# tkkiran/Robust-Conditional-GAN

Hardware: AMD Instinct MI355X
Metric: images/sec G+D train step (CIFAR-10 RCGAN bs=64) (higher is better)
Workload: dtype bf16

## Files before the change

### robust-conditional-gan_amd/cifar.py

```python
import ctypes as C
import os

import warnings

import numpy as np
import torch

from . import _lib as L
from . import ops as O
from .ops_cifar import NO_OPS, Conv2D, Linear, cond_batchnorm, embed_y, spectral_normed_weight
from .runtime import DT, Context, ParamGroup, check_f32_matmul_precision
from .variables import Graph, scoped, variable_scope

Z_DIM = 128
DIM_G = 128
DIM_D = 128
VOCAB_SIZE = 10
EMBEDDING_DIM = 300
IMG_SIZE = 32
IMG_DIM = 3
OUTPUT_DIM = 3072
N_CRITIC = 5
GEN_BS_MULTIPLE = 2
ALGORITHMS = ("rcgan", "rcgan-u", "biased", "unbiased")
# ... 481 lines not shown
            for name, shp, dt in self.feed_layout["d" if steps is not None else key]:
                n = int(np.prod(shp))
                a = np.asarray(arrs[name]).reshape(-1)
                if dt == L.F32:
                    dst[off:off + n].view(np.float32)[:] = a
                else:
                    dst[off:off + n] = a
                off += n
        assert off == words, (off, words)
        with torch.cuda.stream(self.ctx.stream):
            self.feed[key].copy_(ring["slots"][i], non_blocking=True)
            ev = torch.cuda.Event()
            ev.record(self.ctx.stream)
        ring["events"][i] = ev

    def set_feed(self, key, blob):
        src = blob if isinstance(blob, torch.Tensor) else torch.from_numpy(np.ascontiguousarray(blob, dtype=np.int32))
        if src.is_cuda and src.dtype == torch.int32 and src.is_contiguous() and FEED_COPY_KERNEL:
            ctx = self.ctx
            assert src.numel() == self.feed[key].numel(), (src.numel(), self.feed[key].numel())
            ctx.check(ctx.lib.rcgan_copy_words(ctx.h, src.numel(), C.c_void_p(src.data_ptr()), C.c_void_p(self.feed[key].data_ptr())))
            return
        with torch.cuda.stream(self.ctx.stream):
            self.feed[key].copy_(src.reshape(-1), non_blocking=True)

    def _rng(self, t, kind, lo, hi):
        ctx = self.ctx
        ctx.check(ctx.lib.rcgan_rng_fill(ctx.h, t.size, t.dtype, kind, lo, hi, self.seed * 1000003 + self.rank,
                                         C.c_void_p(self.rng_state.data_ptr()), C.c_void_p(t.ptr)))

    def _draw_aug(self, u):
        if self.device_rng:
            ctx = self.ctx
            ctx.check(ctx.lib.rcgan_rng_fill(ctx.h, u.size, u.dtype, 0, 0.0, 1.0, self.seed * 1000003 + self.rank + 700001,
                                             C.c_void_p(self.aug_rng_state.data_ptr()), C.c_void_p(u.ptr)))
        return u

    def _sn_entries(self, conv_update, proj_update):
        ents = []
        for name in self.PD.names:
            if name.endswith("/Filters"):
                ents.append((name, name[:-len("Filters")] + "filters/spectral_norm/u", conv_update))
            elif name.endswith("/W"):
                base = name[:-2]
                upd = conv_update if base.endswith("D.Output") else proj_update
                ents.append((name, base + "/spectral_norm/u", upd))
        return ents

    def _filter_names(self, grp):
        names = []
        pool = fused_pool_d(self.ctx, GEN_BS_MULTIPLE * self.B)
        for n in grp.names:
            if n.endswith("/Filters"):
                shp = grp.shapes[n]
                up = L.CONV_IN_UPSAMPLE2X if (n.startswith("Generator/G.Block.") and n.endswith(".Conv1/Filters")) else 0
                if pool and n in ("Discriminator/D.Block.1.Conv2/Filters", "Discriminator/D.Block.2.Conv2/Filters"):
                    up = L.CONV_OUT_MEANPOOL2
                names.append((n, shp[0], 1, IMG_SIZE if min(shp[2], shp[3]) <= 3 else 8, up))
            elif n == "Generator/G.Input/W" and O.LINEAR_MFMA:
                names.append((n, 1, 1, 1, 0))
        return names

    def _prepare_all(self, which, head_update=False, inputs=None):
        names = []
        for grp in which:
            if grp is not self.PG:
                names += self._filter_names(grp)
        g, embed = self.graph, None
        g.head_E = None
        if self.fused_head and self.PD in which and head_update is not False and self.K <= L.LABELS_NARROW and \
                os.environ.get("RCGAN_HEAD_EMBED_RIDE", "1") == "1":
            _, _, table, w_e, b_e = _head_weights(head_update)
            E = self.ctx.empty((table.shape[0], w_e.param.shape[-1]), L.F32)
            embed = (table, w_e, b_e, E)
        g.trunk_frag = None
        trunk, rf = None, []
        if self.PD in which and self.ctx.act_dtype != L.F32 and (FUSED_TRUNK or O.RF_CONV):
            sn = lambda n: g.sn["Discriminator/%s/Filters" % n][0]
            trunk = [sn("D.Block.%d.%s" % (b, c)) for b in (3, 4, 5, 6) for c in ("Conv1", "Conv2")] if FUSED_TRUNK else None
            if O.RF_CONV:
                d = L.ConvDesc(1, 16, 16, DIM_D, DIM_D, 3, 3, 1, self.ctx.act_dtype, L.CONV_IN_RELU)
                if self.ctx.lib.rcgan_conv_rf_ok(C.byref(d)):
                    rf.append((sn("D.Block.2.Conv1"), d))
        if (trunk or rf) and O.FRAG_IN_PREPARE:
            tf, reqs = O.fragment_requests(self.ctx, trunk, rf)
            rode, written = g.prepare_convs(names, self.ctx.act_dtype, embed=embed, inputs=inputs, frags=reqs)
            if len(written) == len(reqs):
                g.trunk_frag = tf
            else:
                g.trunk_frag = O.fragments_batch(self.ctx, trunk, rf)
        else:
            rode = g.prepare_convs(names, self.ctx.act_dtype, embed=embed, inputs=inputs)
            if trunk or rf:
                g.trunk_frag = O.fragments_batch(self.ctx, trunk, rf)
        if rode and embed is not None:
            g.head_E = embed[3]
        return rode

    def _refresh_generator_filters(self):
        if self._pg_prepared_version != self.PG.version:
            self.graph.refresh_persistent(self._filter_names(self.PG), self.ctx.act_dtype)
            self._pg_prepared_version = self.PG.version

    def confusion_matrix(self):
        ctx = self.ctx
        if self.PC is not None:
            return O.softmax_rows(ctx, self.graph.param("confusion_logits"))
        return self.inp["C_const"]

    def _rides_inputs(self):
        return self.device_rng and self.ride_inputs and self.PD.gradbuf.numel() % 4 == 0

    def _d_body(self, fakes_ready=False):
        ctx, g, B, inp = self.ctx, self.graph, self.B, self.inp
        self._refresh_generator_filters()
        ctx.new_step()
        g.begin_step({1})
        ctx.sn_adam = (dict(group=self.PD, beta1=0.0, beta2=0.9, grad_scale=1.0 / (self.world * self.loss_scale))
                       if (self.fused_tail and ctx.recording and self.PD.hyper is not None) else None)
        g.early_d = self._dp_early(self.PD) if (self.dp_overlap and ctx.recording) else None
        ride = fakes_ready and self._rides_inputs()
        x_all = self.x_all if fakes_ready else ctx.empty((2 * B, OUTPUT_DIM))
        real, fake_dst = x_all.rows(0, B), x_all.rows(B, 2 * B)
        si = None
        if ride:
            fptr, fcount = self.PD.zero_grad(defer=True)
            g.image_pool = ctx.empty((2 * B, 16, 16, 3), x_all.dtype)
            si = L.StepInputsDesc(B, real.dtype, inp["images"].ptr, x_all.ptr, g.image_pool.ptr,
                                  0.0, 1.0 / 128, self.seed * 1000003 + self.rank, self.rng_state.data_ptr(), fptr, fcount,
                                  self.fakes_all.ptr, self.slice_ctr.data_ptr(), N_CRITIC)
        else:
            g.image_pool = None
            self.PD.zero_grad()
            if self.device_rng:
                self._rng(inp["noise"], 0, 0.0, 1.0 / 128)
                if not fakes_ready:
                    self._rng(inp["z"], 1, 0.0, 1.0)
        g.prefetch_sn(self._sn_entries(True, True))
        rode = self._prepare_all((self.PD,) if fakes_ready else (self.PG, self.PD), head_update=None, inputs=si)
        assert rode or si is None, "the step-input rider needs the batched filter preparation"
        if si is None:
            ctx.check(ctx.lib.rcgan_preprocess_cifar(ctx.h, B, inp["images"].ptr, inp["noise"].ptr, real.dtype, real.ptr))
        if fakes_ready:
            fake = self.x_all.rows(B, 2 * B)
        else:
            fake = Generator(B, inp["labels_random"], inp["z"], out=fake_dst)
        d_in = x_all
        if self.aug:
            d_in, g.image_pool = O.diffaugment(ctx, x_all, self._draw_aug(inp["aug_u"]), self.aug, pool=True)
        w = 1.0
        if self.fused_head:
            feat = Discriminator(d_in, None, update_collection=None, _head=False)
            lab_r, lab_f = inp["labels_all"].rows(0, B), inp["labels_all"].rows(B, 2 * B)
            if self.alg == "rcgan-u":
                y_conf = O.gather_rows(ctx, self.confusion_matrix(), inp["labels_random"], B)
                parts = [(B, L.LOSS_HINGE_REAL, inp["labels"], None), (B, L.LOSS_HINGE_FAKE, None, y_conf)]
            elif self.alg == "unbiased":
                parts = [(B, L.LOSS_HINGE_REAL, None, inp["inv_weights"]), (B, L.LOSS_HINGE_FAKE, inp["labels_random"], None)]
            else:
                parts = [(B, L.LOSS_HINGE_REAL, lab_r, None), (B, L.LOSS_HINGE_FAKE, lab_f, None)]
            Discriminator_head(feat, parts, w, self.loss_d, update_collection=None, logits=self.head_logits)
        elif self.alg == "rcgan-u":
            feat_a, wgan_a = Discriminator(d_in, None, update_collection=None)
            feat, wgan = O.rows(ctx, feat_a, 0, B), O.rows(ctx, wgan_a, 0, B)
            feat_f, wgan_f = O.rows(ctx, feat_a, B, 2 * B), O.rows(ctx, wgan_a, B, 2 * B)
            emb = Discriminator_projection(inp["labels"], update_collection=None)
            disc_real = O.proj_logit(ctx, feat, wgan, emb)
            E = Discriminator_projection(inp["arange"], update_collection=None)
            disc_fake = O.proj_logit_all(ctx, feat_f, wgan_f, E)
            y_conf = O.gather_rows(ctx, self.confusion_matrix(), inp["labels_random"], B)
            O.loss_term(ctx, L.LOSS_HINGE_FAKE, disc_fake, w, self.loss_d, wts=y_conf)
            O.loss_term(ctx, L.LOSS_HINGE_REAL, disc_real, w, self.loss_d)
        else:
            feat, wgan = Discriminator(d_in, None, update_collection=None)
            if self.alg in ("biased", "rcgan"):
                emb = Discriminator_projection(inp["labels_all"], update_collection=None)
                disc_all = O.proj_logit(ctx, feat, wgan, emb)
# ... 462 lines not shown
```

### robust-conditional-gan_amd/csrc/conv_mfma.hip

```cpp
#include <vector>
#include "conv_mfma.h"
#include "small_gemm.h"
#include "step_inputs.h"
#include "mfma_util.h"
#include "conv_image.h"
#include "head_rider.h"

#define LDS_PITCH 72
#define WG_PITCH 144



__device__ __forceinline__ void decode_pix(long m, int H, int W, int lh, int lw, int& n, int& oh, int& ow) {
  if (lw >= 0 && lh >= 0) {
    const unsigned mm = (unsigned)m;
    ow = (int)(mm & (unsigned)(W - 1));
    oh = (int)((mm >> lw) & (unsigned)(H - 1));
    n = (int)(mm >> (lw + lh));
  } else {
    ow = (int)(m % W);
    long t = m / W;
    oh = (int)(t % H);
    n = (int)(t / H);
  }
// ... 1037 lines not shown
  long r = idx / Cout;
  int ci = (int)(r % Cin);
  int t = (int)(r / Cin);
  bf16_t v = f32_to_bf16(w[idx] * inv);
  wt[(long)co * T * Cin + (long)t * Cin + ci] = v;
  wd[(long)ci * T * Cout + (long)(T - 1 - t) * Cout + co] = v;
}

struct PhasePrepBatch { struct It { const float* w; const float* sigma; bf16_t* wph; int Cin, Cout, kind; } it[8]; };
__device__ __forceinline__ void phase_taps2(int kind, int ph, int a, int& k0, int& k1) {
  if (kind == 0) { k0 = ph == 0 ? (a == 0 ? 0 : 1) : (a == 0 ? 0 : 2); k1 = ph == 0 ? (a == 0 ? 0 : 2) : (a == 0 ? 1 : 2); }
  else {
    const int u = ph == 0 ? (a == 0 ? 3 : 1) : (a == 0 ? 2 : 0);
    k0 = u == 0 ? 0 : (u == 1 ? 0 : (u == 2 ? 1 : 2)); k1 = u == 0 ? 0 : (u == 1 ? 1 : 2);
  }
}
__device__ __forceinline__ void phase_taps4(int kind, int u, int& k0, int& k1) {
  if (kind == 0) { k0 = u == 0 ? 2 : (u == 1 ? 1 : 0); k1 = u == 0 ? 2 : (u == 1 ? 2 : (u == 2 ? 1 : 0)); }
  else { k0 = u == 0 ? 0 : (u == 1 ? 0 : (u == 2 ? 1 : 2)); k1 = u == 0 ? 0 : (u == 1 ? 1 : 2); }
}

__global__ __launch_bounds__(256) void conv_prepare_phase_kernel(PhasePrepBatch b) {
  const PhasePrepBatch::It it = b.it[blockIdx.y];
  const float inv = (it.sigma ? 1.f / *it.sigma : 1.f) * (it.kind == 1 ? 0.25f : 1.f);
  const long total = 16L * it.Cin * it.Cout;
  bf16_t* const phase_l = it.kind == 0 ? it.wph : it.wph + total;
  bf16_t* const gather_l = it.kind == 0 ? it.wph + total : it.wph;
  const bool fwd_is_phase = it.kind == 0;
  const int Op = fwd_is_phase ? it.Cout : it.Cin, Rp = fwd_is_phase ? it.Cin : it.Cout;
  const int Og = fwd_is_phase ? it.Cin : it.Cout, Rg = fwd_is_phase ? it.Cout : it.Cin;
  for (long e = (long)blockIdx.x * blockDim.x + threadIdx.x; e < total; e += (long)gridDim.x * blockDim.x) {
    {
      const long per = (long)Op * 4 * Rp;
      const int phase = (int)(e / per);
      long r = e - phase * per;
      const int o = (int)(r / (4 * Rp));
      r -= (long)o * 4 * Rp;
      const int ab = (int)(r / Rp), rr = (int)(r - (long)ab * Rp);
      int kh0, kh1, kw0, kw1;
      phase_taps2(it.kind, phase >> 1, ab >> 1, kh0, kh1);
      phase_taps2(it.kind, phase & 1, ab & 1, kw0, kw1);
      const int ci = fwd_is_phase ? rr : o, co = fwd_is_phase ? o : rr;
      float s = 0.f;
      for (int kh = kh0; kh <= kh1; ++kh)
        for (int kw = kw0; kw <= kw1; ++kw) s += it.w[(((long)kh * 3 + kw) * it.Cin + ci) * it.Cout + co];
      phase_l[e] = f32_to_bf16(s * inv);
    }
    {
      const int o = (int)(e / (16L * Rg));
      long r = e - (long)o * 16 * Rg;
      const int uv = (int)(r / Rg), rr = (int)(r - (long)uv * Rg);
      int kh0, kh1, kw0, kw1;
      phase_taps4(it.kind, uv >> 2, kh0, kh1);
      phase_taps4(it.kind, uv & 3, kw0, kw1);
      const int ci = fwd_is_phase ? o : rr, co = fwd_is_phase ? rr : o;
      float s = 0.f;
      for (int kh = kh0; kh <= kh1; ++kh)
        for (int kw = kw0; kw <= kw1; ++kw) s += it.w[(((long)kh * 3 + kw) * it.Cin + ci) * it.Cout + co];
      gather_l[e] = f32_to_bf16(s * inv);
    }
  }
}

int conv_prepare_phase_launch(rcgan_ctx* ctx, int n, const float* const* ws, const float* const* sigmas, bf16_t* const* outs, const int* cins, const int* couts,
                              const int* kinds) {
  for (int base = 0; base < n; base += 8) {
    PhasePrepBatch b;
    const int m = n - base < 8 ? n - base : 8;
    long maxel = 0;
    for (int i = 0; i < m; ++i) {
      b.it[i] = {ws[base + i], sigmas[base + i], outs[base + i], cins[base + i], couts[base + i], kinds[base + i]};
      const long el = 16L * cins[base + i] * couts[base + i];
      if (el > maxel) maxel = el;
    }
    int bx = (int)cdiv(maxel, 256 * 8);
    if (bx > 1024) bx = 1024;
    hipLaunchKernelGGL(conv_prepare_phase_kernel, dim3(bx, m), dim3(256), 0, ctx->stream, b);
    RC_LAUNCH_CHECK(ctx);
  }
  return RCGAN_OK;
}

struct PrepItem { const float* w; const float* sigma; void* out; void* extra; int T, Cin, Cout, mfma, img; };
struct FragRow { int item; int ctn, ss; bf16_t* fwd; bf16_t* bwd; };
struct PrepBatch { PrepItem it[48]; PhasePrepBatch::It ph[8]; FragRow fr[12]; int start[72]; int n, rows, frag_row0, nfrag, gemm_row, inputs_row; SmallGemmArgs gemm; StepInputsArgs inputs; };

static_assert(sizeof(PrepBatch) <= 4096, "kernel arguments are limited to 4 KiB");
constexpr int PREP_MAX_ROWS = (int)(sizeof(PrepBatch::it) / sizeof(PrepItem) + sizeof(PrepBatch::ph) / sizeof(PhasePrepBatch::It) +
                                    sizeof(PrepBatch::fr) / sizeof(FragRow)) + 2;
constexpr int PREP_ROW_STEP = 64;
static_assert(PREP_MAX_ROWS <= 2 * PREP_ROW_STEP, "the row search must reach every row a launch can hold");
static_assert(PREP_MAX_ROWS + 1 <= (int)(sizeof(PrepBatch::start) / sizeof(int)), "start[] holds rows + 1 entries");

__device__ __forceinline__ long frag_index(int row, int k, int ctn, int ss, int nsl) {
  const int blk = row / (16 * ctn), ct = (row - blk * 16 * ctn) >> 4, r = row & 15;
  const int ks = k >> 5, sl = ks / ss, s = ks - sl * ss, kc = (k >> 3) & 3, e = k & 7;
  return ((((long)(blk * nsl + sl) * ss + s) * ctn + ct) * 64 + kc * 16 + r) * 8 + e;
}

__device__ __forceinline__ void prepare_fragment_units(const PrepItem& it, const FragRow& fr, bf16_t (*tile)[66], int bid, int nb) {
  const float inv = it.sigma ? 1.f / *it.sigma : 1.f;
  const int nci = it.Cin / 64, nco = it.Cout / 64;
  const int ntiles = it.T * nci * nco;
  const int nsl_f = it.T * it.Cin / 32 / fr.ss, nsl_d = it.T * it.Cout / 32 / fr.ss;
  const int lane64 = threadIdx.x & 63, grp = threadIdx.x >> 6;
  for (int tl = bid; tl < ntiles; tl += nb) {
    const int cot = tl % nco, cit = (tl / nco) % nci, t = tl / (nco * nci);
    const int ci0 = cit * 64, co0 = cot * 64;
    __syncthreads();
    float v[16];
#pragma unroll
    for (int i = 0; i < 16; ++i) v[i] = it.w[((long)t * it.Cin + ci0 + i * 4 + grp) * it.Cout + co0 + lane64];
#pragma unroll
    for (int i = 0; i < 16; ++i) {
      const int ci = i * 4 + grp;
      const bf16_t h = f32_to_bf16(v[i] * inv);
      fr.bwd[frag_index(ci0 + ci, (it.T - 1 - t) * it.Cout + co0 + lane64, fr.ctn, fr.ss, nsl_d)] = h;
      tile[ci][lane64] = h;
    }
    __syncthreads();
#pragma unroll 4
    for (int i = 0; i < 16; ++i) {
      const int co = i * 4 + grp;
      fr.fwd[frag_index(co0 + co, t * it.Cin + ci0 + lane64, fr.ctn, fr.ss, nsl_f)] = tile[lane64][co];
    }
  }
}

__device__ __forceinline__ void prepare_phase_units(const PhasePrepBatch::It& p, bf16_t (*tile)[66], int bid, int nb) {
  const float inv = (p.sigma ? 1.f / *p.sigma : 1.f) * (p.kind == 1 ? 0.25f : 1.f);
  const long total = 16L * p.Cin * p.Cout;
  bf16_t* const phase_l = p.kind == 0 ? p.wph : p.wph + total;
  bf16_t* const gather_l = p.kind == 0 ? p.wph + total : p.wph;
  const bool fwd_is_phase = p.kind == 0;
  const int nco = p.Cout / 64, units = (p.Cin / 64) * nco * 32;
  const int lane64 = threadIdx.x & 63, grp = threadIdx.x >> 6;
  for (int unit = bid; unit < units; unit += nb) {
    const int cls = unit & 31, tl = unit >> 5, c = cls & 15;
    const int co0 = (tl % nco) * 64, ci0 = (tl / nco) * 64;
    const bool is_phase = cls < 16;
    int kh0, kh1, kw0, kw1;
    if (is_phase) { phase_taps2(p.kind, c >> 3, (c >> 1) & 1, kh0, kh1); phase_taps2(p.kind, (c >> 2) & 1, c & 1, kw0, kw1); }
    else { phase_taps4(p.kind, c >> 2, kh0, kh1); phase_taps4(p.kind, c & 3, kw0, kw1); }
    const bool o_is_co = is_phase ? fwd_is_phase : !fwd_is_phase;
    const int O = o_is_co ? p.Cout : p.Cin, R = o_is_co ? p.Cin : p.Cout;
    bf16_t* const dst = is_phase ? phase_l + (long)(c >> 2) * O * 4 * R + (long)(c & 3) * R : gather_l + (long)c * R;
    const long ostride = is_phase ? 4L * R : 16L * R;
    __syncthreads();
    const float* src[4];
    bool on[4];
#pragma unroll
    for (int j = 0; j < 4; ++j) {
      const int kh = kh0 + (j >> 1), kw = kw0 + (j & 1);
      on[j] = kh <= kh1 && kw <= kw1;
      src[j] = p.w + (((long)(on[j] ? kh * 3 + kw : 0)) * p.Cin + ci0 + grp) * p.Cout + co0 + lane64;
    }
    float v[16][4];
#pragma unroll
    for (int i = 0; i < 16; ++i)
#pragma unroll
      for (int j = 0; j < 4; ++j) v[i][j] = on[j] ? src[j][(long)i * 4 * p.Cout] : 0.f;
#pragma unroll
    for (int i = 0; i < 16; ++i) {
      const int ci = i * 4 + grp;
      float s = 0.f;
#pragma unroll
      for (int j = 0; j < 4; ++j) s += v[i][j];
      const bf16_t h = f32_to_bf16(s * inv);
      if (o_is_co) tile[ci][lane64] = h;
      else dst[(long)(ci0 + ci) * ostride + co0 + lane64] = h;
    }
    if (o_is_co) {
      __syncthreads();
#pragma unroll 4
      for (int i = 0; i < 16; ++i) {
        const int co = i * 4 + grp;
        dst[(long)(co0 + co) * ostride + ci0 + lane64] = tile[lane64][co];
      }
    }
  }
}

__global__ __launch_bounds__(256) void conv_prepare_batch_kernel(PrepBatch b) {
  __shared__ __attribute__((aligned(16))) float lds_u[SG_AS_FLOATS + SG_RED_FLOATS];
  static_assert(sizeof(bf16_t) * 64 * 66 <= sizeof(float) * (SG_AS_FLOATS + SG_RED_FLOATS), "transpose tile fits");
  bf16_t (*tile)[66] = (bf16_t (*)[66])lds_u;
  int row = 0;
#pragma unroll
  for (int step = PREP_ROW_STEP; step > 0; step >>= 1) {
    const int r = row + step;
    if (r < b.rows && (int)blockIdx.x >= b.start[r]) row = r;
  }
  const int bid = (int)blockIdx.x - b.start[row], nb = b.start[row + 1] - b.start[row];
  if (row >= b.frag_row0 && row < b.frag_row0 + b.nfrag) {
    const FragRow fr = b.fr[row - b.frag_row0];
    prepare_fragment_units(b.it[fr.item], fr, tile, bid, nb);
    return;
  }
  if (row == b.gemm_row) { small_gemm_body(b.gemm, bid, lds_u, lds_u + SG_AS_FLOATS); return; }
  if (row == b.inputs_row) { step_inputs_body(b.inputs, bid, nb); return; }
  if (row >= b.n) { prepare_phase_units(b.ph[row - b.n], tile, bid, nb); return; }
  const PrepItem it = b.it[row];
  const long total = (long)it.T * it.Cin * it.Cout;
  const float inv = it.sigma ? 1.f / *it.sigma : 1.f;
  if (it.mfma) {
    bf16_t* wt = (bf16_t*)it.out;
    bf16_t* wd = wt + total;
    const int nci = it.Cin / 64, nco = it.Cout / 64;
    const int ntiles = it.T * nci * nco;
    const int lane64 = threadIdx.x & 63, grp = threadIdx.x >> 6;
    for (int tl = bid; tl < ntiles; tl += nb) {
      const int cot = tl % nco, cit = (tl / nco) % nci, t = tl / (nco * nci);
      const int ci0 = cit * 64, co0 = cot * 64;
      __syncthreads();
      float v[16];
#pragma unroll
      for (int i = 0; i < 16; ++i) v[i] = it.w[((long)t * it.Cin + ci0 + i * 4 + grp) * it.Cout + co0 + lane64];
#pragma unroll
      for (int i = 0; i < 16; ++i) {
        const int ci = i * 4 + grp;
        const bf16_t h = f32_to_bf16(v[i] * inv);
        wd[(long)(ci0 + ci) * it.T * it.Cout + (long)(it.T - 1 - t) * it.Cout + co0 + lane64] = h;
        tile[ci][lane64] = h;
      }
      __syncthreads();
#pragma unroll 4
      for (int i = 0; i < 16; ++i) {
        const int co = i * 4 + grp;
        wt[(long)(co0 + co) * it.T * it.Cin + (long)t * it.Cin + ci0 + lane64] = tile[lane64][co];
      }
    }
    return;
  }
  for (long idx = (long)bid * blockDim.x + threadIdx.x; idx < total; idx += (long)nb * blockDim.x)
    ((float*)it.out)[idx] = it.w[idx] * inv;
  if (it.img) {
    const int cb = it.img == 1 ? it.Cout : it.Cin;
    const long extra = (long)cb * 32 + (long)it.T * 16 * cb;
    for (long e = (long)bid * blockDim.x + threadIdx.x; e < extra; e += (long)nb * blockDim.x)
      ((bf16_t*)it.extra)[e] = img_prepare_elem(e, it.img, it.T, it.Cin, it.Cout, it.w, inv);
  }
}

static int env_int(const char* name, int dflt);
int conv_prepare_batch_launch(rcgan_ctx* ctx, const rcgan_prepare_item* items, int n, const SmallGemmArgs* gemm, const StepInputsArgs* inputs,
                              const rcgan_frag_item* frags, int n_frags) {
  static const int ride = env_int("RCGAN_PREP_PHASE_RIDE", 1);
  std::vector<const float*> pw_, ps_;
  std::vector<bf16_t*> po_;
  std::vector<int> pci, pco, pk;
  for (int i = 0; i < n; ++i) {
    const rcgan_conv_desc& d = items[i].desc;
    if (!mfma_phase_filters(&d)) continue;
    pw_.push_back(items[i].w); ps_.push_back(items[i].sigma);
    po_.push_back((bf16_t*)items[i].prepared + mfma_prepared_sum_fwd(&d));
    pci.push_back(d.cin); pco.push_back(d.cout); pk.push_back((d.flags & RCGAN_CONV_OUT_MEANPOOL2) ? 1 : 0);
  }
  int nride = ride ? (int)pw_.size() : 0;
  if (nride > 8) nride = 8;
  for (int base = 0; base < n; base += 48) {
    PrepBatch b;
    int m = n - base < 48 ? n - base : 48;
    b.n = m;
    const int np = base == 0 ? nride : 0;
    for (int i = 0; i < np; ++i) b.ph[i] = {pw_[i], ps_[i], po_[i], pci[i], pco[i], pk[i]};
    int at = 0;
    for (int i = 0; i < m; ++i) {
      const rcgan_prepare_item& s = items[base + i];
      rcgan_conv_desc d = s.desc;
      b.it[i].w = s.w; b.it[i].sigma = s.sigma; b.it[i].out = s.prepared;
      b.it[i].T = d.kh * d.kw; b.it[i].Cin = d.cin; b.it[i].Cout = d.cout; b.it[i].mfma = mfma_eligible(&d) ? 1 : 0;
      b.it[i].img = b.it[i].mfma ? 0 : img_side(&d);
      b.it[i].extra = b.it[i].img ? (char*)s.prepared + img_extra_offset(&d) : nullptr;
      const long el = (long)d.kh * d.kw * d.cin * d.cout;
      const long img_el = b.it[i].img ? (long)(b.it[i].img == 1 ? d.cout : d.cin) * (32 + b.it[i].T * 16) : 0;
      long want = b.it[i].mfma ? el / 4096 : cdiv(el > img_el ? el : img_el, 256);
      if (want < 1) want = 1;
      if (want > 512) want = 512;
      b.start[i] = at;
      at += (int)want;
    }
    for (int i = 0; i < np; ++i) {
      const long units = (long)(pci[i] / 64) * (pco[i] / 64) * 32;
      b.start[m + i] = at;
      at += units > 1024 ? 1024 : (int)units;
    }
    b.rows = m + np;
    b.frag_row0 = b.rows;
    b.nfrag = 0;
    for (int f = 0; f < n_frags; ++f) {
      const int idx = frags[f].item - base;
      if (idx < 0 || idx >= m) continue;
      const rcgan_conv_desc& d = items[frags[f].item].desc;
      b.fr[b.nfrag] = FragRow{idx, frags[f].ctn, frags[f].ss, (bf16_t*)frags[f].fwd, (bf16_t*)frags[f].bwd};
      b.start[b.rows] = at;
      at += d.kh * d.kw * (d.cin / 64) * (d.cout / 64);
      ++b.nfrag;
      ++b.rows;
    }
    b.start[b.rows] = at;
    b.gemm_row = -1;
    if (gemm && base == 0) {
      b.gemm = *gemm;
      b.gemm_row = b.rows++;
      at += (gemm->d + 15) / 16;
      b.start[b.rows] = at;
    }
    b.inputs_row = -1;
    if (inputs && base == 0) {
      b.inputs = *inputs;
      b.inputs_row = b.rows++;
      const size_t work = (size_t)inputs->n * 3 * 16 * 8 + (inputs->pooled ? (size_t)inputs->n * 768 : 0) + inputs->fill4;
      static const int per = env_int("RCGAN_RIDE_PER_THREAD", 16), cap = env_int("RCGAN_RIDE_MAXWG", 128);
      size_t wgs = (work + 256 * per - 1) / (256 * per);
      if (wgs < 1) wgs = 1;
      if (wgs > (size_t)cap) wgs = cap;
      at += (int)wgs;
      b.start[b.rows] = at;
    }
    hipLaunchKernelGGL(conv_prepare_batch_kernel, dim3(at), dim3(256), 0, ctx->stream, b);
    RC_LAUNCH_CHECK(ctx);
  }
  const int rest = (int)pw_.size() - nride;
  if (rest > 0)
    return conv_prepare_phase_launch(ctx, rest, pw_.data() + nride, ps_.data() + nride, po_.data() + nride, pci.data() + nride, pco.data() + nride,
                                     pk.data() + nride);
  return RCGAN_OK;
}

__global__ void conv_prepare_direct_kernel(const float* w, const float* sigma, float* out, long total) {
  long idx = (long)blockIdx.x * blockDim.x + threadIdx.x;
  if (idx >= total) return;
  const float inv = sigma ? 1.f / *sigma : 1.f;
  out[idx] = w[idx] * inv;
}

static int env_int(const char* name, int dflt) {
  const char* e = getenv(name);
  return e ? atoi(e) : dflt;
}

bool mfma_eligible(const rcgan_conv_desc* d) {
  if (d->dtype != RCGAN_H16) return false;
  if (d->flags & RCGAN_CONV_FORCE_DIRECT) return false;
  if (d->stride != 1) return false;
  if (!((d->kh == 3 && d->kw == 3) || (d->kh == 1 && d->kw == 1))) return false;
  if (d->cin % 64 || d->cout % 64) return false;
  return true;
}

bool mfma_phase_filters(const rcgan_conv_desc* d) {
  return mfma_eligible(d) && (d->flags & (RCGAN_CONV_IN_UPSAMPLE2X | RCGAN_CONV_OUT_MEANPOOL2)) && d->kh == 3 && d->kw == 3;
}

bool mfma_pool_ok(const rcgan_conv_desc* d) {
  static const int on = env_int("RCGAN_FUSED_POOL", 1);
  if (!on || !mfma_phase_filters(d) || !(d->flags & RCGAN_CONV_OUT_MEANPOOL2) || (d->flags & RCGAN_CONV_IN_UPSAMPLE2X)) return false;
  const int lw = ilog2_exact(d->w), lh = ilog2_exact(d->h);
  return lw >= 1 && lh >= 1 && ((long)d->n * (d->h / 2) * (d->w / 2)) % 64 == 0;
}

bool mfma_phase_dgrad_ok(const rcgan_conv_desc* d) {
  static const int on = env_int("RCGAN_UP_PHASE_DGRAD", 1), on1 = env_int("RCGAN_UP_PHASE", 1);
  if (!on || !on1 || !mfma_phase_filters(d)) return false;
  const int lw = ilog2_exact(d->w), lh = ilog2_exact(d->h);
  return lw >= 1 && lh >= 1 && ((long)d->n * (d->h / 2) * (d->w / 2)) % 64 == 0;
}

bool mfma_wgrad_eligible(const rcgan_conv_desc* d) {
  return mfma_eligible(d) && d->cin % 128 == 0 && d->cout % 128 == 0;
}

static int conv_impl() {
  static int v = -1;
  if (v < 0) { const char* e = getenv("RCGAN_CONV_IMPL"); v = (e && e[0] == 'r') ? 0 : 1; }
  return v;
}


template <int BM, int BN, int NS, int KS, int PHASE = 1>
static int launch_conv_glds_phase(rcgan_ctx* ctx, const MfmaConvArgs& a_in) {
  MfmaConvArgs a = a_in;
  a.phase = PHASE;
  static bool attr_set = false;
  size_t lds = (size_t)KS * NS * (BM + BN) * 128;
  const size_t part = (size_t)(KS - 1) * 256 * (BM / 32) * (BN / 32) * 4 * sizeof(float);
  if (part > lds) lds = part;
  if (!attr_set) {
    RC_HIP(ctx, hipFuncSetAttribute((const void*)conv_mfma_glds_kernel<BM, BN, NS, KS, PHASE>, hipFuncAttributeMaxDynamicSharedMemorySize, (int)lds));
    attr_set = true;
  }
  dim3 grid(cdiv(a.M, BM), a.Cout / BN);
  {
    ProfScope ps(ctx, RCGAN_PROF_CONV_MFMA_64, 2.0 * (double)a.M * (PHASE == 2 ? 36 : 9) * a.Cin * a.Cout, 2.0 * (double)a.M * (PHASE == 2 ? 16 : 4) * a.Cin * a.Cout);
    hipLaunchKernelGGL((conv_mfma_glds_kernel<BM, BN, NS, KS, PHASE>), grid, dim3(256 * KS), lds, ctx->stream, a);
  }
  RC_LAUNCH_CHECK(ctx);
  return RCGAN_OK;
}

template <int BM, int BN, int NS, int KS = 1>
static int launch_conv_glds(rcgan_ctx* ctx, const MfmaConvArgs& a) {
// ... 446 lines not shown
```

### robust-conditional-gan_amd/ops.py

```python
import ctypes as C
import os

import torch

from . import _lib as L
from .runtime import DT


def _p(t):
    return C.c_void_p(t.ptr) if t is not None else None


def same_pad(n, k, s):
    out = -(-n // s)
    tot = max((out - 1) * s + k - n, 0)
    return out, tot // 2


def zeros_like_grad(ctx, t):
    g = ctx.empty(t.shape, t.dtype)
    ctx.check(ctx.lib.rcgan_fill_f32(ctx.h, (g.nbytes + 3) // 4, g.ptr, 0.0))
    return g


# ... 39 lines not shown
            buf = DT(ctx.arena.alloc(nbytes), (nbytes,), "u8", ctx.arena.buf)
            ctx.check(ctx.lib.rcgan_conv_prepare(ctx.h, C.byref(desc), _p(self.param), _p(self.sigma), _p(buf)))
            self._prepared[key] = buf
        return self._prepared[key]

    def as_conv1x1(self):
        if self._conv1 is None:
            p = self.param
            pv = DT(p.ptr, (1, 1) + tuple(p.shape), p.dtype, p.base, p.name)
            pv.req, pv.group = p.req, p.group
            if p.grad is not None:
                pv.grad = p.grad.reshape((1, 1) + tuple(p.shape))
            w4 = Weight(self.ctx, pv, self.sigma)
            w4._prepared = self._prepared
            self._conv1 = w4
        return self._conv1

    def grad_target(self):
        if self.sigma is None:
            return self.param.grad
        if self.dwbar is None:
            self.dwbar = DT(self.ctx.arena.alloc(self.param.nbytes), self.param.shape, L.F32, self.ctx.arena.buf)
            self.ctx.check(self.ctx.lib.rcgan_fill_f32(self.ctx.h, self.param.size, self.dwbar.ptr, 0.0))
        return self.dwbar


def prepare_batch(ctx, weights_and_shapes, dtype, persistent=None, embed=None, inputs=None, frags=None):
    todo = []
    index = {}
    for w, k, stride, hw, *rest in weights_and_shapes:
        cin, cout = w.param.shape[-2:]
        desc = L.ConvDesc(1, hw, hw, cin, cout, k, k, stride, dtype, rest[0] if rest else 0)
        nbytes = ctx.lib.rcgan_conv_prepared_bytes(C.byref(desc))
        key = Weight._key(desc, nbytes)
        if persistent is None:
            if key in w._prepared:
                continue
            buf = DT(ctx.arena.alloc(nbytes), (nbytes,), "u8", ctx.arena.buf)
        else:
            slot = persistent.setdefault(w.param.name, {})
            if key not in slot:
                t = torch.empty(int(nbytes), dtype=torch.uint8, device=ctx.device)
                slot[key] = DT(t.data_ptr(), (nbytes,), "u8", t)
            buf = slot[key]
        w._prepared[key] = buf
        index[id(w)] = len(todo)
        todo.append(L.PrepareItem(desc, w.param.ptr, w.sigma.ptr if w.sigma is not None else None, buf.ptr))
    fitems = [(index[id(w)], f, b, ctn, ss, w) for (w, f, b, ctn, ss) in (frags or []) if id(w) in index]
    if todo:
        arr = (L.PrepareItem * len(todo))(*todo)
        if fitems and len(fitems) <= 12:
            ed = si = None
            if embed is not None:
                table, w_e, b_e, E = embed
                v, e_dim = table.shape
                ed = L.EmbedDesc(v, e_dim, w_e.param.shape[-1], table.ptr, w_e.param.ptr, w_e.sigma.ptr if w_e.sigma is not None else None,
                                 b_e.ptr if b_e is not None else None, E.ptr)
            if inputs is not None:
                si = inputs
            fa = (L.FragItem * len(fitems))(*[L.FragItem(i, ctn, ss, f, b) for i, f, b, ctn, ss, _ in fitems])
            ctx.check(ctx.lib.rcgan_conv_prepare_batch_frags(ctx.h, arr, len(todo), C.byref(ed) if ed is not None else None,
                                                             C.byref(si) if si is not None else None, fa, len(fitems)))
            return (embed is not None or inputs is not None), {id(w) for *_, w in fitems}
        if embed is not None or inputs is not None:
            ed = si = None
            if embed is not None:
                table, w_e, b_e, E = embed
                v, e_dim = table.shape
                ed = L.EmbedDesc(v, e_dim, w_e.param.shape[-1], table.ptr, w_e.param.ptr, w_e.sigma.ptr if w_e.sigma is not None else None,
                                 b_e.ptr if b_e is not None else None, E.ptr)
            if inputs is not None:
                si = inputs
            ctx.check(ctx.lib.rcgan_conv_prepare_batch_riders(ctx.h, arr, len(todo), C.byref(ed) if ed is not None else None,
                                                              C.byref(si) if si is not None else None))
            return True if frags is None else (True, set())
        ctx.check(ctx.lib.rcgan_conv_prepare_batch(ctx.h, arr, len(todo)))
    return False if frags is None else (False, set())


RF_CONV = os.environ.get("RCGAN_RF_CONV", "1") != "0"
CONCAT_DIRECT = os.environ.get("RCGAN_CONCAT_DIRECT", "1") != "0"
CONCAT_WGRAD = os.environ.get("RCGAN_CONCAT_WGRAD", "1") != "0"
LINEAR_MFMA = os.environ.get("RCGAN_LINEAR_MFMA", "1") != "0"


FRAG_IN_PREPARE = os.environ.get("RCGAN_FRAG_IN_PREPARE", "0") == "1"


def fragment_requests(ctx, trunk, rf):
    reqs, tf = [], None
    if trunk:
        nb = ctx.lib.rcgan_dtrunk_fragment_bytes()
        tf = DT(ctx.arena.alloc(nb), (nb,), "u8", ctx.arena.buf)
        elems2 = 9 * 128 * 128 * 2
        for i, w in enumerate(trunk):
            reqs.append((w, tf.ptr + i * elems2, tf.ptr + (8 + (7 - i)) * elems2, 2, 36))
    for w, d in rf:
        nb = ctx.lib.rcgan_conv_rf_fragment_bytes(C.byref(d))
        w.rf_frag = DT(ctx.arena.alloc(nb), (nb,), "u8", ctx.arena.buf)
        reqs.append((w, w.rf_frag.ptr, w.rf_frag.ptr + nb // 2, 4, 18))
    return tf, reqs


def fragments_batch(ctx, trunk, rf):
    tp = tf = None
    if trunk:
        tdesc = L.ConvDesc(1, 8, 8, 128, 128, 3, 3, 1, ctx.act_dtype, L.CONV_IN_RELU)
        tp = (C.c_void_p * 8)(*[w.prepared(tdesc).ptr for w in trunk])
        nb = ctx.lib.rcgan_dtrunk_fragment_bytes()
        tf = DT(ctx.arena.alloc(nb), (nb,), "u8", ctx.arena.buf)
    n = len(rf)
    descs = (L.ConvDesc * max(n, 1))(*[d for _, d in rf])
    preps = (C.c_void_p * max(n, 1))(*[w.prepared(d).ptr for w, d in rf])
    frags = []
    for w, d in rf:
        nb = ctx.lib.rcgan_conv_rf_fragment_bytes(C.byref(d))
        w.rf_frag = DT(ctx.arena.alloc(nb), (nb,), "u8", ctx.arena.buf)
        frags.append(w.rf_frag.ptr)
    ctx.check(ctx.lib.rcgan_fragments_prepare(ctx.h, tp, _p(tf), n, descs, preps, (C.c_void_p * max(n, 1))(*frags)))
    return tf


def spectral_norm_batch(ctx, entries):
    n = len(entries)
    if n == 0:
        return []
    items = (L.SnItem * n)()
    weights = []
    saves = []
    for i, (param, u, update) in enumerate(entries):
        c = param.shape[-1]
        k = param.size // c
        sigma = ctx.empty((1,), L.F32)
        save = ctx.empty((ctx.lib.rcgan_sn_save_floats(k, c),), L.F32)
        items[i] = L.SnItem(param.ptr, u.ptr, sigma.ptr, save.ptr, k, c, 1 if update else 0)
        weights.append(Weight(ctx, param, sigma))
        saves.append((save, k, c))
    ctx.check(ctx.lib.rcgan_sn_power_iter(ctx.h, items, n))
    if ctx.recording:
        req = [w for w in weights if w.param.req]
        total = sum((w.param.size + 63) // 64 * 64 for w in req)
        if total and all(w.param.group is not None and w.param.group.sn_scratch and w.param.group.zero_epoch == ctx.epoch for w in req):
            for w in req:
                w.dwbar = w.param.group.dwbar(w.param.name)
        elif total:
            base = ctx.arena.alloc(total * 4)
            ctx.check(ctx.lib.rcgan_fill_f32(ctx.h, total, base, 0.0))
            off = 0
            for w in req:
                w.dwbar = DT(base + off * 4, w.param.shape, L.F32, ctx.arena.buf)
                off += (w.param.size + 63) // 64 * 64

    done = set()

    def bw(only=None):
        ctx.flush_wgrads()
        todo = [(i, w, s) for i, (w, s) in enumerate(zip(weights, saves))
                if i not in done and w.dwbar is not None and w.param.req and (only is None or only(w.param.name))]
        if not todo:
            return
        bi = (L.SnBwdItem * len(todo))()
        for j, (i, w, (save, k, c)) in enumerate(todo):
            bi[j] = L.SnBwdItem(w.param.ptr, w.dwbar.ptr, w.param.grad.ptr, save.ptr, k, c, 1)
            done.add(i)
        fa = getattr(ctx, "sn_adam", None)
        ranges = None
        if fa is not None and not fa.get("done") and len(todo) == len(weights) and all(w.param.group is fa["group"] for _, w, _ in todo):
            grp = fa["group"]
            cover = sorted((grp.offsets[w.param.name], grp.offsets[w.param.name] + w.param.size) for _, w, _ in todo)
# ... 904 lines not shown
```

Measured before the change: 59690.

## Fold fragment copies into weight prepare tiles and vectorize prepare kernels

Fragment layouts for the fused discriminator trunk and the register-file conv are now written from the same tile pass that produces the transposed bf16 filters, and this path becomes the default. That replaces separate fragment rows or a separate fragments_batch launch that re-read the fp32 weights. The prepare and phase kernels switch to 16-byte vector loads and stores, a swizzled double-buffered LDS transpose, and templated phase groups that load the 3x3 taps once per group. The launch order is rotated so the gemm and input rows start first, and new alignment checks are added. Register pressure rises from the v[9][2][8] arrays.

```diff
diff --git a/robust-conditional-gan_amd/cifar.py b/robust-conditional-gan_amd/cifar.py
--- a/robust-conditional-gan_amd/cifar.py
+++ b/robust-conditional-gan_amd/cifar.py
@@ -587,7 +587,7 @@
                 d = L.ConvDesc(1, 16, 16, DIM_D, DIM_D, 3, 3, 1, self.ctx.act_dtype, L.CONV_IN_RELU)
                 if self.ctx.lib.rcgan_conv_rf_ok(C.byref(d)):
                     rf.append((sn("D.Block.2.Conv1"), d))
-        if (trunk or rf) and O.FRAG_IN_PREPARE:
+        if trunk or rf:
             tf, reqs = O.fragment_requests(self.ctx, trunk, rf)
             rode, written = g.prepare_convs(names, self.ctx.act_dtype, embed=embed, inputs=inputs, frags=reqs)
             if len(written) == len(reqs):
@@ -596,8 +596,6 @@
                 g.trunk_frag = O.fragments_batch(self.ctx, trunk, rf)
         else:
             rode = g.prepare_convs(names, self.ctx.act_dtype, embed=embed, inputs=inputs)
-            if trunk or rf:
-                g.trunk_frag = O.fragments_batch(self.ctx, trunk, rf)
         if rode and embed is not None:
             g.head_E = embed[3]
         return rode
diff --git a/robust-conditional-gan_amd/csrc/conv_mfma.hip b/robust-conditional-gan_amd/csrc/conv_mfma.hip
--- a/robust-conditional-gan_amd/csrc/conv_mfma.hip
+++ b/robust-conditional-gan_amd/csrc/conv_mfma.hip
@@ -1143,12 +1143,11 @@
 }
 
 struct PrepItem { const float* w; const float* sigma; void* out; void* extra; int T, Cin, Cout, mfma, img; };
-struct FragRow { int item; int ctn, ss; bf16_t* fwd; bf16_t* bwd; };
-struct PrepBatch { PrepItem it[48]; PhasePrepBatch::It ph[8]; FragRow fr[12]; int start[72]; int n, rows, frag_row0, nfrag, gemm_row, inputs_row; SmallGemmArgs gemm; StepInputsArgs inputs; };
+struct FragRow { int item; int ctn, ss, next; bf16_t* fwd; bf16_t* bwd; };
+struct PrepBatch { PrepItem it[48]; PhasePrepBatch::It ph[8]; FragRow fr[12]; int start[72]; int n, rows, gemm_row, inputs_row, lead; SmallGemmArgs gemm; StepInputsArgs inputs; };
 
 static_assert(sizeof(PrepBatch) <= 4096, "kernel arguments are limited to 4 KiB");
-constexpr int PREP_MAX_ROWS = (int)(sizeof(PrepBatch::it) / sizeof(PrepItem) + sizeof(PrepBatch::ph) / sizeof(PhasePrepBatch::It) +
-                                    sizeof(PrepBatch::fr) / sizeof(FragRow)) + 2;
+constexpr int PREP_MAX_ROWS = (int)(sizeof(PrepBatch::it) / sizeof(PrepItem) + sizeof(PrepBatch::ph) / sizeof(PhasePrepBatch::It)) + 2;
 constexpr int PREP_ROW_STEP = 64;
 static_assert(PREP_MAX_ROWS <= 2 * PREP_ROW_STEP, "the row search must reach every row a launch can hold");
 static_assert(PREP_MAX_ROWS + 1 <= (int)(sizeof(PrepBatch::start) / sizeof(int)), "start[] holds rows + 1 entries");
@@ -1159,136 +1158,188 @@
   return ((((long)(blk * nsl + sl) * ss + s) * ctn + ct) * 64 + kc * 16 + r) * 8 + e;
 }
 
-__device__ __forceinline__ void prepare_fragment_units(const PrepItem& it, const FragRow& fr, bf16_t (*tile)[66], int bid, int nb) {
-  const float inv = it.sigma ? 1.f / *it.sigma : 1.f;
-  const int nci = it.Cin / 64, nco = it.Cout / 64;
-  const int ntiles = it.T * nci * nco;
-  const int nsl_f = it.T * it.Cin / 32 / fr.ss, nsl_d = it.T * it.Cout / 32 / fr.ss;
-  const int lane64 = threadIdx.x & 63, grp = threadIdx.x >> 6;
-  for (int tl = bid; tl < ntiles; tl += nb) {
-    const int cot = tl % nco, cit = (tl / nco) % nci, t = tl / (nco * nci);
-    const int ci0 = cit * 64, co0 = cot * 64;
-    __syncthreads();
-    float v[16];
-#pragma unroll
-    for (int i = 0; i < 16; ++i) v[i] = it.w[((long)t * it.Cin + ci0 + i * 4 + grp) * it.Cout + co0 + lane64];
-#pragma unroll
-    for (int i = 0; i < 16; ++i) {
-      const int ci = i * 4 + grp;
-      const bf16_t h = f32_to_bf16(v[i] * inv);
-      fr.bwd[frag_index(ci0 + ci, (it.T - 1 - t) * it.Cout + co0 + lane64, fr.ctn, fr.ss, nsl_d)] = h;
-      tile[ci][lane64] = h;
-    }
-    __syncthreads();
-#pragma unroll 4
-    for (int i = 0; i < 16; ++i) {
-      const int co = i * 4 + grp;
-      fr.fwd[frag_index(co0 + co, t * it.Cin + ci0 + lane64, fr.ctn, fr.ss, nsl_f)] = tile[lane64][co];
-    }
-  }
-}
-
-__device__ __forceinline__ void prepare_phase_units(const PhasePrepBatch::It& p, bf16_t (*tile)[66], int bid, int nb) {
-  const float inv = (p.sigma ? 1.f / *p.sigma : 1.f) * (p.kind == 1 ? 0.25f : 1.f);
+constexpr int PREP_TILE_DWORDS = 64 * 32;
+
+__device__ __forceinline__ void prep_load8(const float* p, float (&v)[8]) {
+  const float4 a = *(const float4*)p, b = *(const float4*)(p + 4);
+  v[0] = a.x; v[1] = a.y; v[2] = a.z; v[3] = a.w; v[4] = b.x; v[5] = b.y; v[6] = b.z; v[7] = b.w;
+}
+__device__ __forceinline__ uint32_t prep_round16(float x, float inv) {
+  uint32_t h = f32_to_bf16(x * inv);
+#if RCGAN_HALF_FP16
+  asm volatile("" : "+v"(h));
+#endif
+  return h;
+}
+__device__ __forceinline__ uint4 prep_pack8(const float (&v)[8], float inv) {
+  uint4 r;
+  r.x = prep_round16(v[0], inv) | (prep_round16(v[1], inv) << 16);
+  r.y = prep_round16(v[2], inv) | (prep_round16(v[3], inv) << 16);
+  r.z = prep_round16(v[4], inv) | (prep_round16(v[5], inv) << 16);
+  r.w = prep_round16(v[6], inv) | (prep_round16(v[7], inv) << 16);
+  return r;
+}
+__device__ __forceinline__ void prep_store16(bf16_t* p, const uint4& v) { *(uint4*)p = v; }
+__device__ __forceinline__ void prep_tile_put(uint32_t* tile, int rp, int c8, const uint4& r0, const uint4& r1) {
+  const uint32_t a[4] = {r0.x, r0.y, r0.z, r0.w}, b[4] = {r1.x, r1.y, r1.z, r1.w};
+  uint32_t* const row = tile + c8 * 8 * 32 + (rp ^ (c8 << 2));
+#pragma unroll
+  for (int j = 0; j < 4; ++j) {
+    row[(2 * j) * 32] = (a[j] & 0xffffu) | (b[j] << 16);
+    row[(2 * j + 1) * 32] = (a[j] >> 16) | (b[j] & 0xffff0000u);
+  }
+}
+__device__ __forceinline__ uint4 prep_tile_get(const uint32_t* tile, int co, int q) {
+  return *(const uint4*)(tile + co * 32 + ((q ^ ((co >> 3) & 7)) << 2));
+}
+
+constexpr int PHASE_GROUP = 4;
+constexpr int PHASE_GROUPS = 32 / PHASE_GROUP;
+
+template <int KIND, int G>
+__device__ __forceinline__ void prepare_phase_group(const PhasePrepBatch::It& p, uint32_t* lds, int& par, int ci0, int co0, float inv) {
   const long total = 16L * p.Cin * p.Cout;
-  bf16_t* const phase_l = p.kind == 0 ? p.wph : p.wph + total;
-  bf16_t* const gather_l = p.kind == 0 ? p.wph + total : p.wph;
-  const bool fwd_is_phase = p.kind == 0;
-  const int nco = p.Cout / 64, units = (p.Cin / 64) * nco * 32;
-  const int lane64 = threadIdx.x & 63, grp = threadIdx.x >> 6;
+  bf16_t* const phase_l = KIND == 0 ? p.wph : p.wph + total;
+  bf16_t* const gather_l = KIND == 0 ? p.wph + total : p.wph;
+  constexpr bool is_phase = G < 4;
+  constexpr bool o_is_co = is_phase ? KIND == 0 : KIND != 0;
+  const int O = o_is_co ? p.Cout : p.Cin, R = o_is_co ? p.Cin : p.Cout;
+  const long ostride = is_phase ? 4L * R : 16L * R;
+  const int rp = threadIdx.x >> 3, c8 = threadIdx.x & 7;
+  float v[9][2][8];
+  const float* const src = p.w + (long)(ci0 + 2 * rp) * p.Cout + co0 + c8 * 8;
+#pragma unroll
+  for (int t = 0; t < 9; ++t) {
+    prep_load8(src + (long)t * p.Cin * p.Cout, v[t][0]);
+    prep_load8(src + (long)t * p.Cin * p.Cout + p.Cout, v[t][1]);
+  }
+#pragma unroll
+  for (int k = 0; k < PHASE_GROUP; ++k) {
+    const int c = is_phase ? ((((G >> 1) * 2 + (k >> 1)) << 2) | ((G & 1) << 1) | (k & 1)) : (G - 4) * 4 + k;
+    int kh0, kh1, kw0, kw1;
+    if (is_phase) { phase_taps2(KIND, c >> 3, (c >> 1) & 1, kh0, kh1); phase_taps2(KIND, (c >> 2) & 1, c & 1, kw0, kw1); }
+    else { phase_taps4(KIND, c >> 2, kh0, kh1); phase_taps4(KIND, c & 3, kw0, kw1); }
+    bf16_t* const dst = is_phase ? phase_l + (long)(c >> 2) * O * 4 * R + (long)(c & 3) * R : gather_l + (long)c * R;
+    uint4 r[2];
+#pragma unroll
+    for (int h = 0; h < 2; ++h) {
+      float s[8];
+#pragma unroll
+      for (int e = 0; e < 8; ++e) {
+        s[e] = 0.f;
+#pragma unroll
+        for (int j = 0; j < 4; ++j) {
+          const int kh = kh0 + (j >> 1), kw = kw0 + (j & 1);
+          const bool on = kh <= kh1 && kw <= kw1;
+          s[e] += on ? v[on ? kh * 3 + kw : 0][h][e] : 0.f;
+        }
+      }
+      r[h] = prep_pack8(s, inv);
+    }
+    if (!o_is_co) {
+      bf16_t* const d = dst + (long)(ci0 + 2 * rp) * ostride + co0 + c8 * 8;
+      prep_store16(d, r[0]);
+      prep_store16(d + ostride, r[1]);
+    } else {
+      uint32_t* const tile = lds + par * PREP_TILE_DWORDS;
+      par ^= 1;
+      prep_tile_put(tile, rp, c8, r[0], r[1]);
+      __syncthreads();
+#pragma unroll
+      for (int i = 0; i < 2; ++i) {
+        const int co = i * 32 + rp;
+        prep_store16(dst + (long)(co0 + co) * ostride + ci0 + c8 * 8, prep_tile_get(tile, co, c8));
+      }
+    }
+  }
+}
+
+template <int KIND>
+__device__ __forceinline__ void prepare_phase_units(const PhasePrepBatch::It& p, uint32_t* lds, int bid, int nb) {
+  const float inv = (p.sigma ? 1.f / *p.sigma : 1.f) * (KIND == 1 ? 0.25f : 1.f);
+  const int nco = p.Cout / 64, units = (p.Cin / 64) * nco * PHASE_GROUPS;
+  int par = 0;
   for (int unit = bid; unit < units; unit += nb) {
-    const int cls = unit & 31, tl = unit >> 5, c = cls & 15;
+    const int g = unit % PHASE_GROUPS, tl = unit / PHASE_GROUPS;
     const int co0 = (tl % nco) * 64, ci0 = (tl / nco) * 64;
-    const bool is_phase = cls < 16;
-    int kh0, kh1, kw0, kw1;
-    if (is_phase) { phase_taps2(p.kind, c >> 3, (c >> 1) & 1, kh0, kh1); phase_taps2(p.kind, (c >> 2) & 1, c & 1, kw0, kw1); }
-    else { phase_taps4(p.kind, c >> 2, kh0, kh1); phase_taps4(p.kind, c & 3, kw0, kw1); }
-    const bool o_is_co = is_phase ? fwd_is_phase : !fwd_is_phase;
-    const int O = o_is_co ? p.Cout : p.Cin, R = o_is_co ? p.Cin : p.Cout;
-    bf16_t* const dst = is_phase ? phase_l + (long)(c >> 2) * O * 4 * R + (long)(c & 3) * R : gather_l + (long)c * R;
-    const long ostride = is_phase ? 4L * R : 16L * R;
-    __syncthreads();
-    const float* src[4];
-    bool on[4];
-#pragma unroll
-    for (int j = 0; j < 4; ++j) {
-      const int kh = kh0 + (j >> 1), kw = kw0 + (j & 1);
-      on[j] = kh <= kh1 && kw <= kw1;
-      src[j] = p.w + (((long)(on[j] ? kh * 3 + kw : 0)) * p.Cin + ci0 + grp) * p.Cout + co0 + lane64;
-    }
-    float v[16][4];
-#pragma unroll
-    for (int i = 0; i < 16; ++i)
-#pragma unroll
-      for (int j = 0; j < 4; ++j) v[i][j] = on[j] ? src[j][(long)i * 4 * p.Cout] : 0.f;
-#pragma unroll
-    for (int i = 0; i < 16; ++i) {
-      const int ci = i * 4 + grp;
-      float s = 0.f;
-#pragma unroll
-      for (int j = 0; j < 4; ++j) s += v[i][j];
-      const bf16_t h = f32_to_bf16(s * inv);
-      if (o_is_co) tile[ci][lane64] = h;
-      else dst[(long)(ci0 + ci) * ostride + co0 + lane64] = h;
-    }
-    if (o_is_co) {
-      __syncthreads();
-#pragma unroll 4
-      for (int i = 0; i < 16; ++i) {
-        const int co = i * 4 + grp;
-        dst[(long)(co0 + co) * ostride + ci0 + lane64] = tile[lane64][co];
-      }
+    static_assert(PHASE_GROUPS == 8, "one case per group");
+    switch (g) {
+      case 0: prepare_phase_group<KIND, 0>(p, lds, par, ci0, co0, inv); break;
+      case 1: prepare_phase_group<KIND, 1>(p, lds, par, ci0, co0, inv); break;
+      case 2: prepare_phase_group<KIND, 2>(p, lds, par, ci0, co0, inv); break;
+      case 3: prepare_phase_group<KIND, 3>(p, lds, par, ci0, co0, inv); break;
+      case 4: prepare_phase_group<KIND, 4>(p, lds, par, ci0, co0, inv); break;
+      case 5: prepare_phase_group<KIND, 5>(p, lds, par, ci0, co0, inv); break;
+      case 6: prepare_phase_group<KIND, 6>(p, lds, par, ci0, co0, inv); break;
+      default: prepare_phase_group<KIND, 7>(p, lds, par, ci0, co0, inv); break;
     }
   }
 }
 
 __global__ __launch_bounds__(256) void conv_prepare_batch_kernel(PrepBatch b) {
   __shared__ __attribute__((aligned(16))) float lds_u[SG_AS_FLOATS + SG_RED_FLOATS];
-  static_assert(sizeof(bf16_t) * 64 * 66 <= sizeof(float) * (SG_AS_FLOATS + SG_RED_FLOATS), "transpose tile fits");
-  bf16_t (*tile)[66] = (bf16_t (*)[66])lds_u;
+  static_assert(sizeof(uint32_t) * 2 * PREP_TILE_DWORDS <= sizeof(float) * (SG_AS_FLOATS + SG_RED_FLOATS), "two transpose tiles fit");
+  uint32_t* const lds = (uint32_t*)lds_u;
+  const int total_wg = (int)gridDim.x;
+  const int wg = (int)blockIdx.x < b.lead ? total_wg - b.lead + (int)blockIdx.x : (int)blockIdx.x - b.lead;
   int row = 0;
 #pragma unroll
   for (int step = PREP_ROW_STEP; step > 0; step >>= 1) {
     const int r = row + step;
-    if (r < b.rows && (int)blockIdx.x >= b.start[r]) row = r;
-  }
-  const int bid = (int)blockIdx.x - b.start[row], nb = b.start[row + 1] - b.start[row];
-  if (row >= b.frag_row0 && row < b.frag_row0 + b.nfrag) {
-    const FragRow fr = b.fr[row - b.frag_row0];
-    prepare_fragment_units(b.it[fr.item], fr, tile, bid, nb);
-    return;
-  }
+    if (r < b.rows && wg >= b.start[r]) row = r;
+  }
+  const int bid = wg - b.start[row], nb = b.start[row + 1] - b.start[row];
   if (row == b.gemm_row) { small_gemm_body(b.gemm, bid, lds_u, lds_u + SG_AS_FLOATS); return; }
   if (row == b.inputs_row) { step_inputs_body(b.inputs, bid, nb); return; }
-  if (row >= b.n) { prepare_phase_units(b.ph[row - b.n], tile, bid, nb); return; }
+  if (row >= b.n) {
+    const PhasePrepBatch::It& p = b.ph[row - b.n];
+    if (p.kind == 0) prepare_phase_units<0>(p, lds, bid, nb); else prepare_phase_units<1>(p, lds, bid, nb);
+    return;
+  }
   const PrepItem it = b.it[row];
   const long total = (long)it.T * it.Cin * it.Cout;
   const float inv = it.sigma ? 1.f / *it.sigma : 1.f;
-  if (it.mfma) {
+  if (it.mfma & 1) {
     bf16_t* wt = (bf16_t*)it.out;
     bf16_t* wd = wt + total;
     const int nci = it.Cin / 64, nco = it.Cout / 64;
     const int ntiles = it.T * nci * nco;
-    const int lane64 = threadIdx.x & 63, grp = threadIdx.x >> 6;
+    const int rp = threadIdx.x >> 3, c8 = threadIdx.x & 7;
+    const int frag0 = (it.mfma >> 8) - 1;
+    int par = 0;
     for (int tl = bid; tl < ntiles; tl += nb) {
       const int cot = tl % nco, cit = (tl / nco) % nci, t = tl / (nco * nci);
       const int ci0 = cit * 64, co0 = cot * 64;
-      __syncthreads();
-      float v[16];
-#pragma unroll
-      for (int i = 0; i < 16; ++i) v[i] = it.w[((long)t * it.Cin + ci0 + i * 4 + grp) * it.Cout + co0 + lane64];
-#pragma unroll
-      for (int i = 0; i < 16; ++i) {
-        const int ci = i * 4 + grp;
-        const bf16_t h = f32_to_bf16(v[i] * inv);
-        wd[(long)(ci0 + ci) * it.T * it.Cout + (long)(it.T - 1 - t) * it.Cout + co0 + lane64] = h;
-        tile[ci][lane64] = h;
+      float v0[8], v1[8];
+      const float* const src = it.w + ((long)t * it.Cin + ci0 + 2 * rp) * it.Cout + co0 + c8 * 8;
+      prep_load8(src, v0);
+      prep_load8(src + it.Cout, v1);
+      const uint4 r0 = prep_pack8(v0, inv), r1 = prep_pack8(v1, inv);
+      const int kd = (it.T - 1 - t) * it.Cout + co0 + c8 * 8;
+      bf16_t* const d = wd + (long)(ci0 + 2 * rp) * it.T * it.Cout + kd;
+      prep_store16(d, r0);
+      prep_store16(d + (long)it.T * it.Cout, r1);
+      uint32_t* const tile = lds + par * PREP_TILE_DWORDS;
+      par ^= 1;
+      prep_tile_put(tile, rp, c8, r0, r1);
+      for (int f = frag0; f >= 0; f = b.fr[f].next) {
+        const FragRow& fr = b.fr[f];
+        const int nsl_d = it.T * it.Cout / 32 / fr.ss;
+        prep_store16(fr.bwd + frag_index(ci0 + 2 * rp, kd, fr.ctn, fr.ss, nsl_d), r0);
+        prep_store16(fr.bwd + frag_index(ci0 + 2 * rp + 1, kd, fr.ctn, fr.ss, nsl_d), r1);
       }
       __syncthreads();
-#pragma unroll 4
-      for (int i = 0; i < 16; ++i) {
-        const int co = i * 4 + grp;
-        wt[(long)(co0 + co) * it.T * it.Cin + (long)t * it.Cin + ci0 + lane64] = tile[lane64][co];
+      const int kf = t * it.Cin + ci0 + c8 * 8;
+#pragma unroll
+      for (int i = 0; i < 2; ++i) {
+        const int co = i * 32 + rp;
+        const uint4 x = prep_tile_get(tile, co, c8);
+        prep_store16(wt + (long)(co0 + co) * it.T * it.Cin + kf, x);
+        for (int f = frag0; f >= 0; f = b.fr[f].next) {
+          const FragRow& fr = b.fr[f];
+          const int nsl_f = it.T * it.Cin / 32 / fr.ss;
+          prep_store16(fr.fwd + frag_index(co0 + co, kf, fr.ctn, fr.ss, nsl_f), x);
+        }
       }
     }
     return;
@@ -1306,6 +1357,11 @@
 static int env_int(const char* name, int dflt);
 int conv_prepare_batch_launch(rcgan_ctx* ctx, const rcgan_prepare_item* items, int n, const SmallGemmArgs* gemm, const StepInputsArgs* inputs,
                               const rcgan_frag_item* frags, int n_frags) {
+  for (int i = 0; i < n; ++i)
+    RC_REQUIRE(ctx, !mfma_eligible(&items[i].desc) || ((((size_t)items[i].w | (size_t)items[i].prepared) & 15) == 0),
+               "filter %d: weights and prepared buffer must be 16-byte aligned", i);
+  for (int f = 0; f < n_frags; ++f)
+    RC_REQUIRE(ctx, (((size_t)frags[f].fwd | (size_t)frags[f].bwd) & 15) == 0, "fragment copy %d: destinations must be 16-byte aligned", f);
   static const int ride = env_int("RCGAN_PREP_PHASE_RIDE", 1);
   std::vector<const float*> pw_, ps_;
   std::vector<bf16_t*> po_;
@@ -1342,24 +1398,21 @@
       at += (int)want;
     }
     for (int i = 0; i < np; ++i) {
-      const long units = (long)(pci[i] / 64) * (pco[i] / 64) * 32;
+      const long units = (long)(pci[i] / 64) * (pco[i] / 64) * PHASE_GROUPS;
       b.start[m + i] = at;
       at += units > 1024 ? 1024 : (int)units;
     }
     b.rows = m + np;
-    b.frag_row0 = b.rows;
-    b.nfrag = 0;
+    int nfrag = 0;
     for (int f = 0; f < n_frags; ++f) {
       const int idx = frags[f].item - base;
       if (idx < 0 || idx >= m) continue;
-      const rcgan_conv_desc& d = items[frags[f].item].desc;
-      b.fr[b.nfrag] = FragRow{idx, frags[f].ctn, frags[f].ss, (bf16_t*)frags[f].fwd, (bf16_t*)frags[f].bwd};
-      b.start[b.rows] = at;
-      at += d.kh * d.kw * (d.cin / 64) * (d.cout / 64);
-      ++b.nfrag;
-      ++b.rows;
+      b.fr[nfrag] = FragRow{idx, frags[f].ctn, frags[f].ss, (b.it[idx].mfma >> 8) - 1, (bf16_t*)frags[f].fwd, (bf16_t*)frags[f].bwd};
+      b.it[idx].mfma = (b.it[idx].mfma & 1) | ((nfrag + 1) << 8);
+      ++nfrag;
     }
     b.start[b.rows] = at;
+    const int at_items = at;
     b.gemm_row = -1;
     if (gemm && base == 0) {
       b.gemm = *gemm;
@@ -1379,6 +1432,7 @@
       at += (int)wgs;
       b.start[b.rows] = at;
     }
+    b.lead = at - at_items;
     hipLaunchKernelGGL(conv_prepare_batch_kernel, dim3(at), dim3(256), 0, ctx->stream, b);
     RC_LAUNCH_CHECK(ctx);
   }
diff --git a/robust-conditional-gan_amd/ops.py b/robust-conditional-gan_amd/ops.py
--- a/robust-conditional-gan_amd/ops.py
+++ b/robust-conditional-gan_amd/ops.py
@@ -145,9 +145,6 @@
 CONCAT_DIRECT = os.environ.get("RCGAN_CONCAT_DIRECT", "1") != "0"
 CONCAT_WGRAD = os.environ.get("RCGAN_CONCAT_WGRAD", "1") != "0"
 LINEAR_MFMA = os.environ.get("RCGAN_LINEAR_MFMA", "1") != "0"
-
-
-FRAG_IN_PREPARE = os.environ.get("RCGAN_FRAG_IN_PREPARE", "0") == "1"
 
 
 def fragment_requests(ctx, trunk, rf):
```

Result: no change. 60060, median of 6 (+0.6%).
